# sshaoshuai/PointRCNN

Hardware: AMD Instinct MI355X
Metric: KITTI frames/sec, RPN inference end-to-end (16384 pts/frame, bs32 per GPU) (higher is better)
Workload: dtype f32 via split-bf16x6 MFMA (every fp32 operand cut exactly into 3 bf16 pieces, 6 bf16 MFMA products per fp32 product, fp32 accumulate: fp32-grade, measured error 2.9e-7 of sum|x||w| vs 3.0e-7 for the fp32-MFMA kernel; hoisted grouped layers on the split kernel too, unhoisted grouped first layers (xyz; 1 GPU; Full RPN PointNet++ backbone (4 SA-MSG + 4 FP) + cls/reg heads, tools/cfgs/default.yaml, 16384 pts/frame, batch 32 per GPU, random-init weights, eval-mode BN; frames_per_gpu=32, npoints=16384, parallelism=frames sharded, dp1, launch=hipGraph replay, streams=20, hw_queues=4, proposal_layer=normal, clouds=uniform, group_dedup=True, roi_dedup=True

## Files before the change

__graft_entry__.py:

```python
import os
import sys

ROOT = os.path.dirname(os.path.abspath(__file__))
if ROOT not in sys.path:
    sys.path.insert(0, ROOT)


def build():
    from pointrcnn_amd import build as hip_build
    hip_build.build(force=os.path.exists(hip_build.HIPCC), verbose=False)
    import pointrcnn_amd
    pointrcnn_amd.install()
    from pointrcnn_amd import _cabi
    lib = _cabi.lib()
    assert lib.prcnn_abi_version() >= 10
    import oracle
    oracle.build()
    from oracle import stage_reference
    if stage_reference.have_reference():
        stage_reference.stage()
    import pointnet2_lib.pointnet2.pointnet2_modules
    import iou3d_cuda, roipool3d_cuda, pointnet2_cuda


def smoke():
    import numpy as np
    import torch
    import pointrcnn_amd
    pointrcnn_amd.install()
    from pointrcnn_amd import _cabi, ops
    import oracle
    assert torch.cuda.is_available(), "smoke() needs a GPU"
    assert os.path.exists(_cabi.library_path()), "HIP extension missing"
    dev = torch.device("cuda:0")
    cpu = oracle.cpu()
    rng = np.random.default_rng(0)
    T = lambda a: torch.from_numpy(np.ascontiguousarray(a)).to(dev)

    xyz = rng.random((2, 2048, 3), dtype=np.float32)
    fidx = ops.furthest_point_sample(T(xyz), 256)
    assert np.array_equal(fidx.cpu().numpy(), cpu.fps(xyz, 256)), "fps mismatch"
    new_xyz = ops.gather_rows(T(xyz), fidx)
    ia, ib = ops.ball_query2(0.1, 16, 0.2, 32, T(xyz), new_xyz)
    nx = new_xyz.cpu().numpy()
    assert np.array_equal(ia.cpu().numpy(), cpu.ball_query(0.1, 16, xyz, nx)), "ball_query mismatch"
    assert np.array_equal(ib.cpu().numpy(), cpu.ball_query(0.2, 32, xyz, nx)), "ball_query2 mismatch"
    feat = rng.normal(size=(2, 2048, 8)).astype(np.float32)
    w = (rng.normal(size=(32, 11)) * 0.3).astype(np.float32)
# ... 69 lines not shown
```

include/prcnn_pointops.h:

```cpp
#ifndef PRCNN_POINTOPS_H
#define PRCNN_POINTOPS_H

#include <stddef.h>
#include <stdint.h>

#ifdef __cplusplus
extern "C" {
#endif

typedef void* prcnn_stream_t;

#define PRCNN_OK 0
#define PRCNN_EINVAL (-1)
#define PRCNN_EHIP (-2)
#define PRCNN_EUNSUPPORTED (-3)

int prcnn_abi_version(void);
const char* prcnn_last_error(void);
const char* prcnn_build_id(void);


int prcnn_fps(const float* xyz, int B, int N, int npoint, float* tmp, int32_t* idx, prcnn_stream_t stream);

int prcnn_fps_status(void);

#define PRCNN_FPS_ORDER_CANONICAL 0
#define PRCNN_FPS_ORDER_UPSTREAM 1
int prcnn_fps_order(const float* xyz, int B, int N, int npoint, int order, float* tmp, int32_t* idx, prcnn_stream_t stream);

#define PRCNN_ARITH_CANONICAL 0
#define PRCNN_ARITH_UPSTREAM 1
int prcnn_fps_mode(const float* xyz, int B, int N, int npoint, int order, int arith, float* tmp, int32_t* idx, prcnn_stream_t stream);
int prcnn_ball_query_arith(const float* xyz, const float* new_xyz, int B, int N, int M, float radius, int nsample, int arith,
                           int32_t* idx, prcnn_stream_t stream);
int prcnn_three_nn_arith(const float* unknown, const float* known, int B, int n, int m, int arith, float* dist2, int32_t* idx,
                         prcnn_stream_t stream);

int prcnn_gather(const float* feat, const int32_t* idx, int B, int C, int N, int M, float* out, prcnn_stream_t stream);
int prcnn_gather_grad(const float* grad_out, const int32_t* idx, int B, int C, int N, int M, float* grad_feat,
                      prcnn_stream_t stream);

int prcnn_gather_rows(const float* in_cl, int ld_in, const int32_t* idx, int B, int N, int M, int C, float* out,
                      prcnn_stream_t stream);

int prcnn_ball_query(const float* xyz, const float* new_xyz, int B, int N, int M, float radius, int nsample,
                     int32_t* idx, prcnn_stream_t stream);
int prcnn_ball_query2(const float* xyz, const float* new_xyz, int B, int N, int M, float radius_a, int nsample_a,
                      int32_t* idx_a, float radius_b, int nsample_b, int32_t* idx_b, prcnn_stream_t stream);

int prcnn_group(const float* feat, const int32_t* idx, int B, int C, int N, int M, int nsample, float* out,
                prcnn_stream_t stream);
int prcnn_group_grad(const float* grad_out, const int32_t* idx, int B, int C, int N, int M, int nsample,
                     float* grad_feat, prcnn_stream_t stream);

int prcnn_three_nn(const float* unknown, const float* known, int B, int n, int m, float* dist2, int32_t* idx,
// ... 211 lines not shown
```

pointrcnn_amd/_cabi.py:

```python
import ctypes
import os

from . import build as _build

_P = ctypes.c_void_p
_I = ctypes.c_int
_F = ctypes.c_float
_L = ctypes.c_int64
_Z = ctypes.c_size_t
_D = ctypes.c_double



class TrainSrc(ctypes.Structure):
    _fields_ = [("mode", _I), ("rows", _L), ("K", _I),
                ("in_", _P), ("ld_in", _I), ("pro_scale", _P), ("pro_shift", _P),
                ("xyz", _P), ("new_xyz", _P), ("idx", _P), ("feat", _P), ("ld_feat", _I),
                ("B", _I), ("N", _I), ("M", _I), ("ns", _I), ("C", _I),
                ("known", _P), ("idx3", _P), ("w3", _P), ("skip", _P), ("ld_known", _I), ("ld_skip", _I),
                ("n", _I), ("m", _I), ("C2", _I), ("C1", _I),
                ("mult", _P), ("rows_dev", _P), ("norm_rows", _L), ("seg_off", _P), ("seg_cnt", _P), ("row_grp", _P), ("groups", _I)]


class TrainLayer(ctypes.Structure):
    _fields_ = [("Nout", _I), ("W", _P), ("gamma", _P), ("beta", _P), ("eps", _F), ("momentum", _F),
                ("running_mean", _P), ("running_var", _P), ("y", _P), ("cst", _P), ("ld_c", _I), ("wpack", _P), ("wpack_t", _P),
                ("dW", _P), ("dgamma", _P), ("dbeta", _P)]


REQUIRED_ABI = 10

SIGNATURES = {
    "prcnn_abi_version": (_I, []),
    "prcnn_last_error": (ctypes.c_char_p, []),
    "prcnn_build_id": (ctypes.c_char_p, []),
    "prcnn_fps": (_I, [_P, _I, _I, _I, _P, _P, _P]),
    "prcnn_fps_status": (_I, []),
    "prcnn_fps_order": (_I, [_P, _I, _I, _I, _I, _P, _P, _P]),
    "prcnn_fps_mode": (_I, [_P, _I, _I, _I, _I, _I, _P, _P, _P]),
    "prcnn_ball_query_arith": (_I, [_P, _P, _I, _I, _I, _F, _I, _I, _P, _P]),
    "prcnn_three_nn_arith": (_I, [_P, _P, _I, _I, _I, _I, _P, _P, _P]),
    "prcnn_rpn_labels": (_I, [_P, _P, _P, _I, _I, _I, _F, _P, _P, _P]),
    "prcnn_gt_aug_edit": (_I, [_P, _P, _P, _P, _P, _F, _P, _P, _P, _I, _I, _I, _I, _P, _P, _P, _P, _P]),
    "prcnn_corner_iou3d": (_I, [_P, _I, _P, _I, _P, _P, _P]),
    "prcnn_gt_aug_sample": (_I, [_P, _P, _P, _I, _I, _P, _P, _P, _I, _P, _I, _P, _I, _P, _P, _I, _I, ctypes.c_uint32,
                                 _P, _P, _P, _P, _P, _P, _P, _P]),
    "prcnn_host_pts_in_boxes3d": (_I, [_P, _P, _L, _L, _P]),
    "prcnn_host_roipool3d": (_I, [_P, _P, _P, _L, _L, _L, _L, _P, _P, _P]),
    "prcnn_gather": (_I, [_P, _P, _I, _I, _I, _I, _P, _P]),
    "prcnn_gather_grad": (_I, [_P, _P, _I, _I, _I, _I, _P, _P]),
    "prcnn_gather_rows": (_I, [_P, _I, _P, _I, _I, _I, _I, _P, _P]),
    "prcnn_ball_query": (_I, [_P, _P, _I, _I, _I, _F, _I, _P, _P]),
    "prcnn_ball_query2": (_I, [_P, _P, _I, _I, _I, _F, _I, _P, _F, _I, _P, _P]),
    "prcnn_group": (_I, [_P, _P, _I, _I, _I, _I, _I, _P, _P]),
    "prcnn_group_grad": (_I, [_P, _P, _I, _I, _I, _I, _I, _P, _P]),
    "prcnn_three_nn": (_I, [_P, _P, _I, _I, _I, _P, _P, _P, _P]),
    "prcnn_three_interp": (_I, [_P, _P, _P, _I, _I, _I, _I, _P, _P]),
    "prcnn_three_interp_grad": (_I, [_P, _P, _P, _I, _I, _I, _I, _P, _P, _P]),
    "prcnn_wpack_floats": (_Z, [_I, _I]),
    "prcnn_pack_weight": (_I, [_P, _I, _I, _I, _P, _P]),
    "prcnn_mlp_rows": (_I, [_P, _I, _L, _I, _P, _P, _I, _I, _P, _I, _I, _I, _P, _I, _P, _I, _P]),
    "prcnn_mlp_group": (_I, [_P, _P, _P, _P, _I, _I, _I, _I, _I, _I, _P, _P, _P, _P, _I, _I, _P, _I, _I, _I, _P, _P]),
    "prcnn_mlp_group_split": (_I, [_P, _P, _P, _P, _I, _I, _I, _I, _I, _I, _P, _P, _P, _P, _I, _P, _I, _I, _P, _I, _I, _I, _P, _P]),
    "prcnn_mlp_interp": (_I, [_P, _I, _P, _P, _P, _I, _I, _I, _I, _I, _I, _P, _P, _P, _I, _I, _P, _I, _I, _P]),
    "prcnn_mlp_rows_addinterp": (_I, [_P, _I, _I, _P, _P, _I, _I, _P, _I, _P, _P, _I, _I, _I, _P, _I, _I, _P]),
    "prcnn_wsplit_bytes": (_Z, [_I, _I]),
    "prcnn_pack_weight_split": (_I, [_P, _I, _I, _I, _P, _P]),
    "prcnn_mlp_chain_interp_split": (_I, [_P, _I, _P, _P, _I, _I, _I, _I, _P, _P, _P, _P, _I, _I, _I, _P, _I, _I, _P]),
    "prcnn_mlp_chain_rows_split": (_I, [_P, _I, _L, _I, _P, _P, _P, _P, _P, _I, _P, _I, _I, _P]),
# ... 54 lines not shown
    pass


def library_path():
    return _build.LIB


def lib():
    global _lib
    if _lib is not None:
        return _lib
    import torch
    path = _build.LIB
    if not os.path.exists(path):
        try:
            _build.build(verbose=False)
        except Exception as e:
            raise PointOpsError(
                "libprcnn_pointops.so is missing and could not be built (%s). The HIP extension is "
                "mandatory: there is no CPU fallback. Run `python -m pointrcnn_amd.build`." % e)
    elif not os.environ.get("PRCNN_POINTOPS_LIB") and _build.have_sources() and _build.library_id(path) != _build.source_id():
        if not os.path.exists(_build.HIPCC):
            raise PointOpsError("%s is stale (built from %s, sources are %s) and hipcc is not available to rebuild it"
                                % (path, _build.library_id(path), _build.source_id()))
        try:
            _build.build(verbose=False)
        except Exception as e:
            raise PointOpsError("%s is stale and could not be rebuilt (%s)" % (path, e))
    try:
        handle = ctypes.CDLL(path)
    except OSError as e:
        raise PointOpsError("cannot load %s: %s" % (path, e))
    handle.prcnn_abi_version.restype = _I
    if handle.prcnn_abi_version() < REQUIRED_ABI:
        raise PointOpsError("%s implements ABI %d, this binding needs %d (include/prcnn_pointops.h)"
                            % (path, handle.prcnn_abi_version(), REQUIRED_ABI))
    for name, (res, args) in SIGNATURES.items():
        fn = getattr(handle, name)
        fn.restype = res
        fn.argtypes = args
    _lib = handle
    return handle


EUNSUPPORTED = -3


def check(rc, what=""):
    if rc != 0:
        msg = lib().prcnn_last_error()
        raise PointOpsError("%s failed (code %d): %s" % (what or "prcnn call", rc, msg.decode() if msg else "?"))
```

pointrcnn_amd/csrc/cabi_common.hip:

```cpp
#include "common.h"
#include <stdarg.h>

static thread_local char g_err[512] = "";

int prcnn_fail(int code, const char* fmt, ...) {
    va_list ap;
    va_start(ap, fmt);
    vsnprintf(g_err, sizeof(g_err), fmt, ap);
    va_end(ap);
    return code;
}

PRCNN_API const char* prcnn_last_error(void) { return g_err; }
PRCNN_API int prcnn_abi_version(void) { return 10; }

#ifndef PRCNN_BUILD_ID
#define PRCNN_BUILD_ID "PRCNN_BUILD_ID=unknown"
#endif
PRCNN_API const char* prcnn_build_id(void) { return &PRCNN_BUILD_ID[sizeof("PRCNN_BUILD_ID=") - 1]; }
```

pointrcnn_amd/csrc/fps.hip:

```cpp
#include "lds_sort.h"

typedef float f32x2 __attribute__((ext_vector_type(2)));
template <int PPT> struct fvec_t { typedef float type __attribute__((ext_vector_type(PPT))); };
template <> struct fvec_t<1> { typedef float type __attribute__((ext_vector_type(2))); };

#define FPS_DPP_MAX(v, ctrl) asm volatile("s_nop 1\n\tv_max_i32_dpp %0, %0, %0 " ctrl : "+v"(v))

__device__ __forceinline__ int wave_max_i32_fused(int v) {
    FPS_DPP_MAX(v, "row_shr:1 row_mask:0xf bank_mask:0xf");
    FPS_DPP_MAX(v, "row_shr:2 row_mask:0xf bank_mask:0xf");
    FPS_DPP_MAX(v, "row_shr:4 row_mask:0xf bank_mask:0xf");
    FPS_DPP_MAX(v, "row_shr:8 row_mask:0xf bank_mask:0xf");
    FPS_DPP_MAX(v, "row_bcast:15 row_mask:0xa bank_mask:0xf");
    FPS_DPP_MAX(v, "row_bcast:31 row_mask:0xc bank_mask:0xf");
    asm volatile("s_nop 1");
    return __builtin_amdgcn_readlane(v, 63);
}
__device__ __forceinline__ int row0_max_i32_fused(int v) {
    FPS_DPP_MAX(v, "row_shr:1 row_mask:0xf bank_mask:0xf");
    FPS_DPP_MAX(v, "row_shr:2 row_mask:0xf bank_mask:0xf");
    FPS_DPP_MAX(v, "row_shr:4 row_mask:0xf bank_mask:0xf");
    FPS_DPP_MAX(v, "row_shr:8 row_mask:0xf bank_mask:0xf");
    asm volatile("s_nop 1");
    return __builtin_amdgcn_readlane(v, 15);
// ... 73 lines not shown
                     "s_nop 1\n\t"
                     : [t] "=&v"(t), [acc] "=&v"(acc), [sa] "=&s"(sa), [sb] "=&s"(sb)
                     : [best] "v"(best), [p0] "v"(pt[0]), [p1] "v"(pt[1]), [p2] "v"(pt[2]), [p3] "v"(pt[3])
                     : "vcc");
        eqbits = acc;
        return t;
    }
};

#define FPS_EQ2(pa, pb) "v_cmp_eq_f32_e64 %[sa], " pa ", %[best]\n\tv_cmp_eq_f32_e64 %[sb], " pb ", %[best]\n\t"
#define FPS_AC2 "v_addc_co_u32_e64 %[a0], vcc, %[a0], %[a0], %[sa]\n\tv_addc_co_u32_e64 %[a1], vcc, %[a1], %[a1], %[sb]\n\t"
template <class V> __device__ __forceinline__ int wave_max_eq2_16(const V& pt, float best, unsigned& eqbits) {
    int t; unsigned a0, a1; unsigned long long sa, sb, sc, sd;
    asm volatile("v_mov_b32 %[t], %[best]\n\tv_mov_b32 %[a0], 0\n\tv_mov_b32 %[a1], 0\n\t"
                 FPS_EQ2("%[p15]", "%[p7]") FPS_D1 FPS_AC2
                 FPS_EQ2("%[p14]", "%[p6]") FPS_D2 FPS_AC2
                 FPS_EQ2("%[p13]", "%[p5]") FPS_D3 FPS_AC2
                 FPS_EQ2("%[p12]", "%[p4]") FPS_D4 FPS_AC2
                 FPS_EQ2("%[p11]", "%[p3]") FPS_D5 FPS_AC2
                 FPS_EQ2("%[p10]", "%[p2]") FPS_D6 FPS_AC2
                 FPS_EQ2("%[p9]", "%[p1]")
                 "v_cmp_eq_f32_e64 %[sc], %[p8], %[best]\n\tv_cmp_eq_f32_e64 %[sd], %[p0], %[best]\n\t"
                 FPS_AC2
                 "v_addc_co_u32_e64 %[a0], vcc, %[a0], %[a0], %[sc]\n\tv_addc_co_u32_e64 %[a1], vcc, %[a1], %[a1], %[sd]\n\t"
                 : [t] "=&v"(t), [a0] "=&v"(a0), [a1] "=&v"(a1), [sa] "=&s"(sa), [sb] "=&s"(sb), [sc] "=&s"(sc), [sd] "=&s"(sd)
                 : [best] "v"(best), [p0] "v"(pt[0]), [p1] "v"(pt[1]), [p2] "v"(pt[2]), [p3] "v"(pt[3]), [p4] "v"(pt[4]), [p5] "v"(pt[5]),
                   [p6] "v"(pt[6]), [p7] "v"(pt[7]), [p8] "v"(pt[8]), [p9] "v"(pt[9]), [p10] "v"(pt[10]), [p11] "v"(pt[11]),
                   [p12] "v"(pt[12]), [p13] "v"(pt[13]), [p14] "v"(pt[14]), [p15] "v"(pt[15])
                 : "vcc");
    eqbits = (a0 << 8) | a1;
    return t;
}

template <int BLOCK, int PPT>
__global__ __launch_bounds__(BLOCK) void fps_reg_kernel(const float* __restrict__ xyz, int N, int npoint,
                                                        int32_t* __restrict__ idx_out) {
    constexpr int NW = BLOCK / 64;
    typedef typename fvec_t<PPT>::type fvec;
    __shared__ float slot[2][NW][8];

    const int b = blockIdx.x;
    const int tid = threadIdx.x;
    const int lane = tid & 63;
    const int wave = tid >> 6;
    const float* __restrict__ p = xyz + (size_t)b * N * 3;
    int32_t* __restrict__ out = idx_out + (size_t)b * npoint;

    fvec px, py, pz, pt;
#pragma unroll
    for (int i = 0; i < PPT; i++) {
        int k = tid * PPT + i;
        bool ok = k < N;
        px[i] = ok ? p[k * 3 + 0] : 0.f;
        py[i] = ok ? p[k * 3 + 1] : 0.f;
        pz[i] = ok ? p[k * 3 + 2] : 0.f;
        pt[i] = ok ? 1e10f : -1.0f;
    }
    if (tid == 0 && npoint > 0) out[0] = 0;
    float x0 = p[0], y0 = p[1], z0 = p[2];

    for (int j = 1; j < npoint; j++) {
        float best = -2.0f;
        if (PPT >= 2) {
            const f32x2 qx = {x0, x0}, qy = {y0, y0}, qz = {z0, z0};
#pragma unroll
            for (int i = 0; i + 1 < PPT; i += 2) {
                f32x2 dx = (f32x2){px[i], px[i + 1]} - qx;
                f32x2 dy = (f32x2){py[i], py[i + 1]} - qy;
                f32x2 dz = (f32x2){pz[i], pz[i + 1]} - qz;
// ... 31 lines not shown
            }
            __syncthreads();
            const float* r = slot[j & 1][lane < NW ? lane : 0];
            int v = lane < NW ? __float_as_int(r[0]) : (int)0x80000000;
            int id = __float_as_int(r[1]);
            float rx = r[2], ry = r[3], rz = r[4];
            const int gmax = row0_max_i32_fused(v);
            const int wwin = __builtin_ctzll(__ballot(v == gmax));
            gidx = __builtin_amdgcn_readlane(id, wwin);
            x0 = __int_as_float(__builtin_amdgcn_readlane(__float_as_int(rx), wwin));
            y0 = __int_as_float(__builtin_amdgcn_readlane(__float_as_int(ry), wwin));
            z0 = __int_as_float(__builtin_amdgcn_readlane(__float_as_int(rz), wwin));
        }
        if (tid == 0) out[j] = gidx;
    }
}

#define FPS_BIG 1.0e18f
#ifndef FPS_V
#define FPS_V 6
#endif
#ifndef FPS_PAIR_ASM
#define FPS_PAIR_ASM 1
#endif

__device__ __forceinline__ unsigned morton_spread6(unsigned v) {
    v &= 0x3fu;
    v = (v | (v << 8)) & 0x0000300fu;
    v = (v | (v << 4)) & 0x000030c3u;
    v = (v | (v << 2)) & 0x00009249u;
    return v;
}

__global__ __launch_bounds__(1024) void fps_sort_kernel(const float* __restrict__ xyz, int N, int NP, int32_t* __restrict__ perm) {
    extern __shared__ unsigned keys[];
    __shared__ float red[6][16];
    const int b = blockIdx.x, tid = threadIdx.x, lane = tid & 63, wave = tid >> 6, nw = blockDim.x >> 6;
    const float* __restrict__ p = xyz + (size_t)b * N * 3;
    float lo[3] = {FPS_BIG, FPS_BIG, FPS_BIG}, hi[3] = {-FPS_BIG, -FPS_BIG, -FPS_BIG};
    for (int k = tid; k < N; k += blockDim.x)
#pragma unroll
        for (int a = 0; a < 3; a++) { float v = p[k * 3 + a]; lo[a] = fminf(lo[a], v); hi[a] = fmaxf(hi[a], v); }
#pragma unroll
    for (int a = 0; a < 3; a++) {
        for (int o = 32; o > 0; o >>= 1) { lo[a] = fminf(lo[a], __shfl_xor(lo[a], o)); hi[a] = fmaxf(hi[a], __shfl_xor(hi[a], o)); }
        if (lane == 0) { red[a][wave] = lo[a]; red[3 + a][wave] = hi[a]; }
    }
    __syncthreads();
    float scale[3];
#pragma unroll
    for (int a = 0; a < 3; a++) {
        float l = red[a][0], h = red[3 + a][0];
        for (int w = 1; w < nw; w++) { l = fminf(l, red[a][w]); h = fmaxf(h, red[3 + a][w]); }
        lo[a] = l;
        scale[a] = (h > l) ? 63.0f / (h - l) : 0.f;
    }
    unsigned v[16];
    if (tid * 16 < NP) {
#pragma unroll
        for (int e = 0; e < 16; e++) {
            const int k = tid * 16 + e;
            unsigned key = ~0u;
            if (k < N) {
                unsigned qx = (unsigned)((p[k * 3 + 0] - lo[0]) * scale[0]);
                unsigned qy = (unsigned)((p[k * 3 + 1] - lo[1]) * scale[1]);
                unsigned qz = (unsigned)((p[k * 3 + 2] - lo[2]) * scale[2]);
                unsigned m = (morton_spread6(qx) << 2) | (morton_spread6(qz) << 1) | morton_spread6(qy);
// ... 50 lines not shown
}
__device__ __forceinline__ void fps_xt_publish(unsigned (*xt)[64], int cb, int wave, const fps_cand_t& c) {
    unsigned* t = xt[cb];
    t[wave] = __float_as_uint(c.x); t[16 + wave] = __float_as_uint(c.y); t[32 + wave] = __float_as_uint(c.z);
    asm volatile("ds_max_u64 %0, %1 offset:192" : : "v"((unsigned)(size_t)&t[0]), "v"(c.key) : "memory");
    if (wave == 0) *(unsigned long long*)&xt[cb == 2 ? 0 : cb + 1][48] = 0ULL;
}
__device__ __forceinline__ int fps_xt_collect(unsigned (*xt)[64], int cb, int lane, float& x0, float& y0, float& z0, int& wl) {
    const int tv = (int)xt[cb][lane];
    const unsigned klo = (unsigned)__builtin_amdgcn_readlane(tv, 48);
    wl = (int)(klo & 15u);
    x0 = __int_as_float(__builtin_amdgcn_readlane(tv, wl));
    y0 = __int_as_float(__builtin_amdgcn_readlane(tv, wl | 16));
    z0 = __int_as_float(__builtin_amdgcn_readlane(tv, wl | 32));
    return (int)(0xFFFFFFFu - (klo >> 4));
}

#ifdef PRCNN_FPS_TIMING
__device__ unsigned long long prcnn_fps_dbg[16 * 8 + 16 + 16 * 16];
PRCNN_API int prcnn_fps_timing_read(unsigned long long* host_out) {
    return hipMemcpyFromSymbol(host_out, HIP_SYMBOL(prcnn_fps_dbg), sizeof(prcnn_fps_dbg)) == hipSuccess ? 0 : -1;
}
#define FPS_T(...) __VA_ARGS__
#ifndef PRCNN_FPS_TIMING_WAVE
#define PRCNN_FPS_TIMING_WAVE -1
#endif
#define FPS_NOW(w) ((PRCNN_FPS_TIMING_WAVE < 0 || (w) == PRCNN_FPS_TIMING_WAVE) ? __builtin_readcyclecounter() : 0ULL)
#else
#define FPS_T(...)
#endif

template <int PPT>
__global__ __launch_bounds__(1024) void fps_pruned_kernel(const float* __restrict__ xyz, const int32_t* __restrict__ perm,
                                                          int N, int npoint, int32_t* __restrict__ idx_out) {
    constexpr int BLOCK = 1024, NW = 16;
    typedef typename fvec_t<PPT>::type fvec;
    FPS_XT_DECL;
    extern __shared__ int s_po[];
    __builtin_amdgcn_s_setprio(2);

    const int b = blockIdx.x, tid = threadIdx.x, lane = tid & 63, wave = tid >> 6;
    const int wave_u = __builtin_amdgcn_readfirstlane(wave);
    const float* __restrict__ p = xyz + (size_t)b * N * 3;
    const int32_t* __restrict__ pm = perm + (size_t)b * N;
    int32_t* __restrict__ out = idx_out + (size_t)b * npoint;

    fvec px, py, pz, pt;
    float lox = FPS_BIG, loy = FPS_BIG, loz = FPS_BIG, hix = -FPS_BIG, hiy = -FPS_BIG, hiz = -FPS_BIG;
#pragma unroll
    for (int i = 0; i < PPT; i++) {
        int s = tid * PPT + i;
        bool ok = s < N;
        int o = ok ? pm[s] : 0x7fffffff;
        s_po[i * BLOCK + tid] = o;
        px[i] = ok ? p[o * 3 + 0] : 0.f;
        py[i] = ok ? p[o * 3 + 1] : 0.f;
        pz[i] = ok ? p[o * 3 + 2] : 0.f;
        pt[i] = ok ? 1e10f : -1.0f;
        if (ok) {
            lox = fminf(lox, px[i]); hix = fmaxf(hix, px[i]);
            loy = fminf(loy, py[i]); hiy = fmaxf(hiy, py[i]);
            loz = fminf(loz, pz[i]); hiz = fmaxf(hiz, pz[i]);
        }
    }
    lox = wave_min_f32_fused(lox); loy = wave_min_f32_fused(loy); loz = wave_min_f32_fused(loz);
    hix = wave_max_f32_fused(hix); hiy = wave_max_f32_fused(hiy); hiz = wave_max_f32_fused(hiz);

// ... 78 lines not shown
                cy = __int_as_float(__builtin_amdgcn_readlane(__float_as_int(by), owner));
                cz = __int_as_float(__builtin_amdgcn_readlane(__float_as_int(bz), owner));
            }
            cval = wmaxf;
            first = false;
            fps_cand_set(cand, wave, cx, cy, cz, cval, corig);
            FPS_T(t_u4 += __builtin_readcyclecounter() - u3;)
            }
            __builtin_amdgcn_s_setprio(2);
        }
#if FPS_V & 2
        else __builtin_amdgcn_s_setprio(2);
#endif
        FPS_T(unsigned long long t1 = __builtin_readcyclecounter(); t_upd += t1 - t0; n_upd += update ? 1 : 0;)
        if (lane == 0) fps_xt_publish(xt, cb, wave, cand);
        __syncthreads();
        FPS_T(unsigned long long t2 = __builtin_readcyclecounter(); t_wait += t2 - t1;)
        int wwin;
        const int gorig = fps_xt_collect(xt, cb, lane, x0, y0, z0, wwin);
#if FPS_V & 2
        if ((unsigned)(wave_u - wwin + 1) <= 2u) __builtin_amdgcn_s_setprio(3);
#endif
        wprev = wwin;
        cb = cb == 2 ? 0 : cb + 1;
        if (tid == 0) out[j] = gorig;
        FPS_T(t0 = __builtin_readcyclecounter(); t_red += t0 - t2;)
    }
    FPS_T(if (b == 0 && lane == 0) { unsigned long long* d = prcnn_fps_dbg + wave * 8; d[0] = t_upd; d[1] = t_wait; d[2] = t_red; d[3] = n_upd;
                                     d[4] = __builtin_readcyclecounter() - t_begin; d[5] = t_u1; d[6] = t_u2; d[7] = t_u3; prcnn_fps_dbg[128 + wave] = t_u4; })
}

template <int PPT, int NW>
__global__ __launch_bounds__(NW * 64) void fps_slot_kernel(const float* __restrict__ xyz, const int32_t* __restrict__ perm,
                                                          int N, int npoint, int32_t* __restrict__ idx_out) {
    constexpr int BLOCK = NW * 64;
    typedef typename fvec_t<PPT>::type fvec;
    FPS_XT_DECL;
    extern __shared__ int s_po[];
    __builtin_amdgcn_s_setprio(2);

    const int b = blockIdx.x, tid = threadIdx.x, lane = tid & 63, wave = tid >> 6;
    const int wave_u = __builtin_amdgcn_readfirstlane(wave);
    const float* __restrict__ p = xyz + (size_t)b * N * 3;
    const int32_t* __restrict__ pm = perm + (size_t)b * N;
    int32_t* __restrict__ out = idx_out + (size_t)b * npoint;

    fvec px, py, pz, pt;
    float lox = FPS_BIG, loy = FPS_BIG, loz = FPS_BIG, hix = -FPS_BIG, hiy = -FPS_BIG, hiz = -FPS_BIG;
#pragma unroll
    for (int i = 0; i < PPT; i++) {
        int s = (wave * PPT + i) * 64 + lane;
        bool ok = s < N;
        int o = ok ? pm[s] : 0x7fffffff;
        s_po[i * BLOCK + tid] = o;
        px[i] = ok ? p[o * 3 + 0] : 0.f;
        py[i] = ok ? p[o * 3 + 1] : 0.f;
        pz[i] = ok ? p[o * 3 + 2] : 0.f;
        pt[i] = ok ? 1e10f : -1.0f;
        if (ok) {
            lox = fminf(lox, px[i]); hix = fmaxf(hix, px[i]);
            loy = fminf(loy, py[i]); hiy = fmaxf(hiy, py[i]);
            loz = fminf(loz, pz[i]); hiz = fmaxf(hiz, pz[i]);
        }
    }
    lox = wave_min_f32_fused(lox); loy = wave_min_f32_fused(loy); loz = wave_min_f32_fused(loz);
    hix = wave_max_f32_fused(hix); hiy = wave_max_f32_fused(hiy); hiz = wave_max_f32_fused(hiz);

// ... 136 lines not shown
        }
#if FPS_V & 2
        else __builtin_amdgcn_s_setprio(2);
#endif
        FPS_T(unsigned long long q4 = FPS_NOW(wave);)
        if (lane == 0) fps_xt_publish(xt, cb, wave, cand);
        __syncthreads();
        FPS_T(unsigned long long q5 = FPS_NOW(wave); q_pub += q5 - q4;)
        int wwin;
        const int gorig = fps_xt_collect(xt, cb, lane, x0, y0, z0, wwin);
#if FPS_V & 2
        if ((unsigned)(wave_u - wwin + 1) <= 2u) __builtin_amdgcn_s_setprio(3);
#endif
        wprev = wwin;
        cb = cb == 2 ? 0 : cb + 1;
        if (tid == 0) out[j] = gorig;
        FPS_T(q0 = FPS_NOW(wave); q_coll += q0 - q5;)
    }
    FPS_T(if (b == 0 && lane == 0) { unsigned long long* d = prcnn_fps_dbg + 144 + wave * 16; d[0] = q_test; d[1] = q_dist; d[2] = q_max; d[3] = q_search; d[4] = q_pub;
                                     d[5] = q_coll; d[6] = q_nupd; d[7] = q_npair; d[8] = FPS_NOW(wave) - q_begin; })
}

struct fps_bcand_t { float x, y, z, v, s; unsigned orig, mask; unsigned long long key; };
__device__ __forceinline__ void fps_bcand_set(fps_bcand_t& c, int wave, float cx, float cy, float cz, float cval, float csec, int corig, unsigned cmask) {
    const unsigned hi = (unsigned)__float_as_int(cval) ^ 0x80000000u;
    const unsigned o = (unsigned)min(corig, 0xFFFFFFF);
    c.x = cx; c.y = cy; c.z = cz; c.v = cval; c.s = csec; c.orig = o; c.mask = cmask; c.key = ((unsigned long long)hi << 32) | ((0xFFFFFFFu - o) << 4) | (unsigned)wave;
    asm volatile("" : "+v"(c.x), "+v"(c.y), "+v"(c.z), "+v"(c.v), "+v"(c.s), "+v"(c.orig), "+v"(c.mask), "+v"(c.key));
}
#define FPS_BT_WORDS 160

template <int PPT, int NW>
__global__ __launch_bounds__(NW * 64) void fps_batch_kernel(const float* __restrict__ xyz, const int32_t* __restrict__ perm,
                                                           int N, int npoint, int32_t* __restrict__ idx_out) {
    static_assert(NW == 16 && PPT == 16, "rows of 16 lanes = the 16 waves; 8 pair boxes");
    constexpr int BLOCK = NW * 64;
    typedef typename fvec_t<PPT>::type fvec;
    typedef float f32x4 __attribute__((ext_vector_type(4)));
    typedef unsigned u32x4 __attribute__((ext_vector_type(4)));
    __shared__ __attribute__((aligned(256))) unsigned xt[3][FPS_BT_WORDS];
    __shared__ __attribute__((aligned(32))) float wbox[16][8];
    extern __shared__ int s_po[];
    __builtin_amdgcn_s_setprio(2);

    const int b = blockIdx.x, tid = threadIdx.x, lane = tid & 63, wave = tid >> 6, l15 = lane & 15;
    const int wave_u = __builtin_amdgcn_readfirstlane(wave);
    const float* __restrict__ p = xyz + (size_t)b * N * 3;
    const int32_t* __restrict__ pm = perm + (size_t)b * N;
    int32_t* __restrict__ out = idx_out + (size_t)b * npoint;

    fvec px, py, pz, pt;
    float lox = FPS_BIG, loy = FPS_BIG, loz = FPS_BIG, hix = -FPS_BIG, hiy = -FPS_BIG, hiz = -FPS_BIG;
#pragma unroll
    for (int i = 0; i < PPT; i++) {
        int s = (wave * PPT + i) * 64 + lane;
        bool ok = s < N;
        int o = ok ? pm[s] : 0x7fffffff;
        s_po[i * BLOCK + tid] = o;
        px[i] = ok ? p[o * 3 + 0] : 0.f;
        py[i] = ok ? p[o * 3 + 1] : 0.f;
        pz[i] = ok ? p[o * 3 + 2] : 0.f;
        pt[i] = ok ? 1e10f : -1.0f;
        if (ok) {
            lox = fminf(lox, px[i]); hix = fmaxf(hix, px[i]);
            loy = fminf(loy, py[i]); hiy = fmaxf(hiy, py[i]);
            loz = fminf(loz, pz[i]); hiz = fmaxf(hiz, pz[i]);
        }
// ... 294 lines not shown
    __shared__ int sval[2][NW], sidx[2][NW];
    const int b = blockIdx.x, tid = threadIdx.x, lane = tid & 63, wave = tid >> 6;
    const float* __restrict__ p = xyz + (size_t)b * N * 3;
    float* __restrict__ t = tmp + (size_t)b * N;
    int32_t* __restrict__ out = idx_out + (size_t)b * npoint;
    for (int k = tid; k < N; k += 1024) t[k] = 1e10f;
    if (tid == 0 && npoint > 0) out[0] = 0;
    int old = 0;
    for (int j = 1; j < npoint; j++) {
        float x0 = p[old * 3], y0 = p[old * 3 + 1], z0 = p[old * 3 + 2];
        float best = -2.0f;
        int bk = 0x7fffffff;
        for (int k = tid; k < N; k += 1024) {
            float d = sqdist3(p[k * 3], p[k * 3 + 1], p[k * 3 + 2], x0, y0, z0);
            float v = t[k];
            v = d < v ? d : v;
            t[k] = v;
            if (v > best) { best = v; bk = k; }
        }
        int vb = __float_as_int(best);
        int wmax = wave_max_i32(vb);
        int widx = wave_min_i32(vb == wmax ? bk : 0x7fffffff);
        if (lane == 0) { sval[j & 1][wave] = wmax; sidx[j & 1][wave] = widx; }
        __syncthreads();
        int v = lane < NW ? sval[j & 1][lane] : (int)0x80000000;
        int id = lane < NW ? sidx[j & 1][lane] : 0x7fffffff;
        int gmax = row0_max_i32(v);
        old = row0_min_i32(v == gmax ? id : 0x7fffffff);
        if (tid == 0) out[j] = old;
    }
}

template <int BLOCK, int PPT>
static void launch_fps(const float* xyz, int B, int N, int npoint, int32_t* idx, hipStream_t s) {
    hipLaunchKernelGGL((fps_reg_kernel<BLOCK, PPT>), dim3(B), dim3(BLOCK), 0, s, xyz, N, npoint, idx);
}

static int* fps_timeout_word() {
    static int* word = [] {
        int* w = nullptr;
        if (hipHostMalloc((void**)&w, sizeof(int), hipHostMallocMapped) != hipSuccess) { (void)hipGetLastError(); return (int*)nullptr; }
        *w = 0;
        return w;
    }();
    return word;
}

PRCNN_API int prcnn_fps_status(void) {
    int* w = fps_timeout_word();
    if (w && __atomic_exchange_n(w, 0, __ATOMIC_RELAXED) != 0)
        return prcnn_fail(PRCNN_EHIP, "prcnn_fps: a multi-workgroup launch (N > 16384) gave up waiting for a partner slice; "
                                      "its output holds -1 indices (were all ceil(N/16384) workgroups of a frame able to become resident?)");
    return PRCNN_OK;
}

PRCNN_API int prcnn_fps(const float* xyz, int B, int N, int npoint, float* tmp, int32_t* idx, prcnn_stream_t stream) {
    PRCNN_REQUIRE(B >= 0 && N > 0 && npoint >= 0, "prcnn_fps: bad shape B=%d N=%d npoint=%d", B, N, npoint);
    PRCNN_REQUIRE(npoint <= N, "prcnn_fps: npoint %d > N %d", npoint, N);
    if (B == 0 || npoint == 0) return PRCNN_OK;
    PRCNN_REQUIRE(xyz && idx, "prcnn_fps: null pointer");
    hipStream_t s = (hipStream_t)stream;
    if (tmp && N > 2048 && N <= 16384) {
        int NP = 1;
        while (NP < N) NP <<= 1;
        int32_t* perm = reinterpret_cast<int32_t*>(tmp);
        static PrcnnLdsLimit sort_attr;
        if (!sort_attr.raise((const void*)fps_sort_kernel, 80 * 1024))
            return prcnn_fail(PRCNN_EHIP, "prcnn_fps: cannot raise the dynamic LDS limit of the sort kernel");
        const int sort_threads = NP / 16 < 64 ? 64 : NP / 16;
        hipLaunchKernelGGL(fps_sort_kernel, dim3(B), dim3(sort_threads), lds_sort_bytes(NP, sizeof(unsigned)), s, xyz, N, NP, perm);
        PRCNN_LAUNCH_CHECK("prcnn_fps(sort)");
        static PrcnnLdsLimit pruned_attr;
        if (!pruned_attr.raise((const void*)fps_pruned_kernel<16>, 16 * 4096))
            return prcnn_fail(PRCNN_EHIP, "prcnn_fps: cannot raise the dynamic LDS limit of the pruned kernel");
        const char* slots_env = getenv("PRCNN_FPS_SLOTS");
        const bool slots = slots_env == nullptr || atoi(slots_env) != 0;
        static PrcnnLdsLimit slot_attr;
        if (slots && N > 8192 && !slot_attr.raise((const void*)fps_slot_kernel<16, 16>, 16 * 4096))
            return prcnn_fail(PRCNN_EHIP, "prcnn_fps: cannot raise the dynamic LDS limit of the slot kernel");
        const char* batch_env = getenv("PRCNN_FPS_BATCH");
        const bool batch = batch_env != nullptr && atoi(batch_env) != 0;
        static PrcnnLdsLimit batch_attr;
        if (slots && batch && N > 8192 && !batch_attr.raise((const void*)fps_batch_kernel<16, 16>, 16 * 4096))
            return prcnn_fail(PRCNN_EHIP, "prcnn_fps: cannot raise the dynamic LDS limit of the batch kernel");
        if (slots && batch && N > 8192) hipLaunchKernelGGL((fps_batch_kernel<16, 16>), dim3(B), dim3(1024), 16 * 4096, s, xyz, perm, N, npoint, idx);
        else if (slots && N > 8192) hipLaunchKernelGGL((fps_slot_kernel<16, 16>), dim3(B), dim3(1024), 16 * 4096, s, xyz, perm, N, npoint, idx);
        else if (N <= 4096) hipLaunchKernelGGL((fps_pruned_kernel<4>), dim3(B), dim3(1024), 4 * 4096, s, xyz, perm, N, npoint, idx);
        else if (N <= 8192) hipLaunchKernelGGL((fps_pruned_kernel<8>), dim3(B), dim3(1024), 8 * 4096, s, xyz, perm, N, npoint, idx);
        else hipLaunchKernelGGL((fps_pruned_kernel<16>), dim3(B), dim3(1024), 16 * 4096, s, xyz, perm, N, npoint, idx);
    }
    else if (N <= 64) launch_fps<64, 1>(xyz, B, N, npoint, idx, s);
    else if (N <= 128) launch_fps<64, 2>(xyz, B, N, npoint, idx, s);
    else if (N <= 256) launch_fps<64, 4>(xyz, B, N, npoint, idx, s);
    else if (N <= 512) launch_fps<64, 8>(xyz, B, N, npoint, idx, s);
    else if (N <= 1024) launch_fps<64, 16>(xyz, B, N, npoint, idx, s);
    else if (N <= 2048) launch_fps<256, 8>(xyz, B, N, npoint, idx, s);
    else if (N <= 4096) launch_fps<256, 16>(xyz, B, N, npoint, idx, s);
    else if (N <= 8192) launch_fps<1024, 8>(xyz, B, N, npoint, idx, s);
    else if (N <= 16384) launch_fps<1024, 16>(xyz, B, N, npoint, idx, s);
    else {
        PRCNN_REQUIRE(tmp, "prcnn_fps: N=%d > 16384 needs the (B,N) tmp buffer", N);
        const int S = prcnn_divup(N, FPS_MULTI_SLICE);
        static const bool use_mem = getenv("PRCNN_FPS_MEM") != nullptr;
        if (!use_mem && S <= FPS_MULTI_MAX_SPLIT && ((uintptr_t)tmp & 7) == 0) {
            const size_t slot_bytes = (size_t)B * 2 * S * 5 * sizeof(unsigned long long);
            if (prcnn_fill_words(tmp, 0xFFFFFFFFu, slot_bytes / 4, s) != hipSuccess) return prcnn_fail(PRCNN_EHIP, "prcnn_fps: cannot clear the exchange slots");
            if (int st = prcnn_fps_status()) return st;
            hipLaunchKernelGGL(fps_multi_kernel, dim3(B * S), dim3(1024), 0, s, xyz, N, npoint, S, reinterpret_cast<unsigned long long*>(tmp), idx,
                               fps_timeout_word());
        } else {
            hipLaunchKernelGGL(fps_mem_kernel, dim3(B), dim3(1024), 0, s, xyz, N, npoint, tmp, idx);
        }
    }
    PRCNN_LAUNCH_CHECK("prcnn_fps");
    return PRCNN_OK;
}

__global__ __launch_bounds__(1024) void fps_upstream_order_kernel(const float* __restrict__ xyz, int N, int npoint, int T,
                                                                  float* __restrict__ tmp, int32_t* __restrict__ idx_out) {
    constexpr int NWMAX = 16;
    __shared__ int sval[2][NWMAX], stid[2][NWMAX], sidx[2][NWMAX];
    const int b = blockIdx.x, tid = threadIdx.x, lane = tid & 63, wave = tid >> 6;
    const int nw = (blockDim.x + 63) >> 6;
    const float* __restrict__ p = xyz + (size_t)b * N * 3;
    float* __restrict__ t = tmp + (size_t)b * N;
    int32_t* __restrict__ out = idx_out + (size_t)b * npoint;
    for (int k = tid; k < N; k += blockDim.x) t[k] = 1e10f;
    if (tid == 0 && npoint > 0) out[0] = 0;
    __syncthreads();
    int old = 0;
    for (int j = 1; j < npoint; j++) {
        const float x0 = p[old * 3], y0 = p[old * 3 + 1], z0 = p[old * 3 + 2];
        float best = -2.0f;
        int bk = 0x7fffffff;
        if (tid < T) {
            for (int k = tid; k < N; k += T) {
                const float d = sqdist3(p[k * 3], p[k * 3 + 1], p[k * 3 + 2], x0, y0, z0);
                float v = t[k];
                v = d < v ? d : v;
                t[k] = v;
                if (v > best) { best = v; bk = k; }
            }
        }
        const int vb = __float_as_int(best);
        const int wmax = wave_max_i32(vb);
        const int wtid = wave_min_i32(vb == wmax ? tid : 0x7fffffff);
        const int wk = __shfl(bk, wtid & 63);
        if (lane == 0) { sval[j & 1][wave] = wmax; stid[j & 1][wave] = wtid; sidx[j & 1][wave] = wk; }
// ... 26 lines not shown
```

pointrcnn_amd/ops.py:

```python
import ctypes
import os
import threading

import torch

from . import _cabi

_INT = torch.int32
_F32 = torch.float32
FPS_PRUNED = os.environ.get("PRCNN_FPS_PRUNED", "1") == "1"


def _stream():
    return torch.cuda.current_stream().cuda_stream


def _chk(t, name, dtype=_F32, ndim=None):
    if not isinstance(t, torch.Tensor):
        raise TypeError("%s must be a torch.Tensor" % name)
    if not t.is_cuda:
        raise RuntimeError("%s must be a CUDA(HIP) tensor: the HIP kernels are the only implementation" % name)
    if t.dtype != dtype:
        raise RuntimeError("%s must have dtype %s, got %s" % (name, dtype, t.dtype))
    if not t.is_contiguous():
        raise RuntimeError("%s must be contiguous" % name)
    if ndim is not None and t.dim() != ndim:
        raise RuntimeError("%s must have %d dims, got shape %s" % (name, ndim, tuple(t.shape)))
    return t


def _p(t):
    return None if t is None else t.data_ptr()


def furthest_point_sample(xyz, npoint, order="canonical"):
    _chk(xyz, "xyz", ndim=3)
    B, N, _ = xyz.shape
    idx = torch.empty((B, npoint), dtype=_INT, device=xyz.device)
    if order != "canonical":
        if order != "upstream":
            raise ValueError("furthest_point_sample: order must be 'canonical' or 'upstream'")
        tmp = torch.empty((B, N), dtype=_F32, device=xyz.device)
        _cabi.check(_cabi.lib().prcnn_fps_order(_p(xyz), B, N, npoint, 1, _p(tmp), _p(idx), _stream()), "prcnn_fps_order")
        return idx
    tmp = torch.empty((B, N), dtype=_F32, device=xyz.device) if (N > 16384 or (N > 2048 and FPS_PRUNED)) else None
    L = _cabi.lib()
    _cabi.check(L.prcnn_fps(_p(xyz), B, N, npoint, _p(tmp), _p(idx), _stream()), "prcnn_fps")
    return idx


_ARITH = {"canonical": 0, "upstream": 1}
_ORDER = {"canonical": 0, "upstream": 1}


def furthest_point_sample_mode(xyz, npoint, order="canonical", arith="canonical"):
    _chk(xyz, "xyz", ndim=3)
    B, N, _ = xyz.shape
    idx = torch.empty((B, npoint), dtype=_INT, device=xyz.device)
    tmp = torch.empty((B, N), dtype=_F32, device=xyz.device)
    _cabi.check(_cabi.lib().prcnn_fps_mode(_p(xyz), B, N, npoint, _ORDER[order], _ARITH[arith], _p(tmp), _p(idx), _stream()), "prcnn_fps_mode")
    return idx


def ball_query_arith(radius, nsample, xyz, new_xyz, arith="upstream"):
    _chk(xyz, "xyz", ndim=3); _chk(new_xyz, "new_xyz", ndim=3)
    B, N, _ = xyz.shape
    M = new_xyz.shape[1]
    idx = torch.empty((B, M, nsample), dtype=_INT, device=xyz.device)
    _cabi.check(_cabi.lib().prcnn_ball_query_arith(_p(xyz), _p(new_xyz), B, N, M, float(radius), nsample, _ARITH[arith], _p(idx), _stream()),
                "prcnn_ball_query_arith")
    return idx


def three_nn_arith(unknown, known, arith="upstream"):
    _chk(unknown, "unknown", ndim=3); _chk(known, "known", ndim=3)
    B, n, _ = unknown.shape
    m = known.shape[1]
    d2 = torch.empty((B, n, 3), dtype=_F32, device=unknown.device)
    idx = torch.empty((B, n, 3), dtype=_INT, device=unknown.device)
    _cabi.check(_cabi.lib().prcnn_three_nn_arith(_p(unknown), _p(known), B, n, m, _ARITH[arith], _p(d2), _p(idx), _stream()),
                "prcnn_three_nn_arith")
    return d2, idx


def fps_status():
    _cabi.check(_cabi.lib().prcnn_fps_status(), "prcnn_fps_status")


def gather(features, idx):
    _chk(features, "features", ndim=3); _chk(idx, "idx", _INT, 2)
    B, C, N = features.shape
    M = idx.shape[1]
    out = torch.empty((B, C, M), dtype=_F32, device=features.device)
    _cabi.check(_cabi.lib().prcnn_gather(_p(features), _p(idx), B, C, N, M, _p(out), _stream()), "prcnn_gather")
    return out


def gather_grad(grad_out, idx, N):
    _chk(grad_out, "grad_out", ndim=3); _chk(idx, "idx", _INT, 2)
    B, C, M = grad_out.shape
    g = torch.zeros((B, C, N), dtype=_F32, device=grad_out.device)
    _cabi.check(_cabi.lib().prcnn_gather_grad(_p(grad_out), _p(idx), B, C, N, M, _p(g), _stream()), "prcnn_gather_grad")
    return g


def gather_rows(in_cl, idx):
    _chk(idx, "idx", _INT, 2)
    B, N, C = in_cl.shape
    M = idx.shape[1]
    out = torch.empty((B, M, C), dtype=_F32, device=in_cl.device)
    _cabi.check(_cabi.lib().prcnn_gather_rows(_p(in_cl), _row_stride(in_cl), _p(idx), B, N, M, C, _p(out), _stream()),
                "prcnn_gather_rows")
    return out


GRID_MIN_POINTS = 2048 if os.environ.get("PRCNN_GRID_SEARCH", "1") != "0" else 1 << 62
THREE_NN_GRID_MIN = int(os.environ.get("PRCNN_THREE_NN_GRID_MIN", "1024")) if GRID_MIN_POINTS < (1 << 62) else 1 << 62
DENSE_SCAN = os.environ.get("PRCNN_DENSE_SCAN", "1") != "0"
BQ_GRID_CELLS = int(os.environ.get("PRCNN_BQ_GRID_CELLS", "128"))


class Grid:

    def __init__(self, xyz, min_cell=0.0, cells_per_axis=64):
        _chk(xyz, "xyz", ndim=3)
        self.B, self.N = xyz.shape[0], xyz.shape[1]
        L = _cabi.lib()
        nbytes = L.prcnn_grid_bytes(self.B, self.N)
        self.buf = torch.empty((max(nbytes, 16),), dtype=torch.uint8, device=xyz.device)
        _cabi.check(L.prcnn_grid_build(_p(xyz), self.B, self.N, float(min_cell), int(cells_per_axis), _p(self.buf), nbytes, _stream()),
                    "prcnn_grid_build")


def ball_query_grid(grid, new_xyz, radius_a, nsample_a, radius_b=0.0, nsample_b=0, xyz=None):
    _chk(new_xyz, "new_xyz", ndim=3)
    B, M = new_xyz.shape[0], new_xyz.shape[1]
    if B != grid.B:
        raise ValueError("ball_query_grid: %d frames of centroids vs %d frames in the grid" % (B, grid.B))
    ia = torch.empty((B, M, nsample_a), dtype=_INT, device=new_xyz.device)
    ib = torch.empty((B, M, nsample_b), dtype=_INT, device=new_xyz.device) if nsample_b else None
    _cabi.check(_cabi.lib().prcnn_ball_query2_grid(_p(grid.buf), _p(xyz), _p(new_xyz), B, grid.N, M, float(radius_a), nsample_a, _p(ia),
                                                   float(radius_b), nsample_b, _p(ib), _stream()), "prcnn_ball_query2_grid")
    return (ia, ib) if nsample_b else ia


# ... 723 lines not shown
```

Before: 13870 frames/s.

## Skip nested FPS on already FPS-ordered inputs via a prefix validity check

Sampled xyz produced by gather_rows from an FPS index is tagged as FPS-ordered. A later furthest-point sample on such a set takes a nested path. A parallel prefix kernel writes the identity order, checks each point's minimum distance to earlier points for zeros or out-of-range values, and sets a per-frame flag. The existing FPS kernels read the flag and return early for frames whose prefix passed, which avoids the sequential FPS loop on the deeper SA levels. The cost is an extra kernel, a flag fill, and reliance on tagging that is tied to tensor versions.

```diff
diff --git a/__graft_entry__.py b/__graft_entry__.py
--- a/__graft_entry__.py
+++ b/__graft_entry__.py
@@ -13,7 +13,7 @@
     pointrcnn_amd.install()
     from pointrcnn_amd import _cabi
     lib = _cabi.lib()
-    assert lib.prcnn_abi_version() >= 10
+    assert lib.prcnn_abi_version() >= 11
     import oracle
     oracle.build()
     from oracle import stage_reference
diff --git a/include/prcnn_pointops.h b/include/prcnn_pointops.h
--- a/include/prcnn_pointops.h
+++ b/include/prcnn_pointops.h
@@ -21,6 +21,8 @@
 
 
 int prcnn_fps(const float* xyz, int B, int N, int npoint, float* tmp, int32_t* idx, prcnn_stream_t stream);
+
+int prcnn_fps_nested(const float* xyz, int B, int N, int npoint, float* tmp, int32_t* flags, int32_t* idx, prcnn_stream_t stream);
 
 int prcnn_fps_status(void);
 
diff --git a/pointrcnn_amd/_cabi.py b/pointrcnn_amd/_cabi.py
--- a/pointrcnn_amd/_cabi.py
+++ b/pointrcnn_amd/_cabi.py
@@ -29,12 +29,14 @@
 
 
 REQUIRED_ABI = 10
+ABI_SINCE = {"prcnn_fps_nested": 11}
 
 SIGNATURES = {
     "prcnn_abi_version": (_I, []),
     "prcnn_last_error": (ctypes.c_char_p, []),
     "prcnn_build_id": (ctypes.c_char_p, []),
     "prcnn_fps": (_I, [_P, _I, _I, _I, _P, _P, _P]),
+    "prcnn_fps_nested": (_I, [_P, _I, _I, _I, _P, _P, _P, _P]),
     "prcnn_fps_status": (_I, []),
     "prcnn_fps_order": (_I, [_P, _I, _I, _I, _I, _P, _P, _P]),
     "prcnn_fps_mode": (_I, [_P, _I, _I, _I, _I, _I, _P, _P, _P]),
@@ -155,9 +157,10 @@
     except OSError as e:
         raise PointOpsError("cannot load %s: %s" % (path, e))
     handle.prcnn_abi_version.restype = _I
-    if handle.prcnn_abi_version() < REQUIRED_ABI:
+    need = max([REQUIRED_ABI] + list(ABI_SINCE.values()))
+    if handle.prcnn_abi_version() < need:
         raise PointOpsError("%s implements ABI %d, this binding needs %d (include/prcnn_pointops.h)"
-                            % (path, handle.prcnn_abi_version(), REQUIRED_ABI))
+                            % (path, handle.prcnn_abi_version(), need))
     for name, (res, args) in SIGNATURES.items():
         fn = getattr(handle, name)
         fn.restype = res
diff --git a/pointrcnn_amd/csrc/cabi_common.hip b/pointrcnn_amd/csrc/cabi_common.hip
--- a/pointrcnn_amd/csrc/cabi_common.hip
+++ b/pointrcnn_amd/csrc/cabi_common.hip
@@ -12,7 +12,7 @@
 }
 
 PRCNN_API const char* prcnn_last_error(void) { return g_err; }
-PRCNN_API int prcnn_abi_version(void) { return 10; }
+PRCNN_API int prcnn_abi_version(void) { return 11; }
 
 #ifndef PRCNN_BUILD_ID
 #define PRCNN_BUILD_ID "PRCNN_BUILD_ID=unknown"
diff --git a/pointrcnn_amd/csrc/fps.hip b/pointrcnn_amd/csrc/fps.hip
--- a/pointrcnn_amd/csrc/fps.hip
+++ b/pointrcnn_amd/csrc/fps.hip
@@ -129,9 +129,12 @@
     return t;
 }
 
+#define FPS_SKIP_FRAME(skip) do { if ((skip) != nullptr && (skip)[blockIdx.x] != 0) return; } while (0)
+
 template <int BLOCK, int PPT>
 __global__ __launch_bounds__(BLOCK) void fps_reg_kernel(const float* __restrict__ xyz, int N, int npoint,
-                                                        int32_t* __restrict__ idx_out) {
+                                                        int32_t* __restrict__ idx_out, const int32_t* __restrict__ skip) {
+    FPS_SKIP_FRAME(skip);
     constexpr int NW = BLOCK / 64;
     typedef typename fvec_t<PPT>::type fvec;
     __shared__ float slot[2][NW][8];
@@ -229,7 +232,9 @@
     return v;
 }
 
-__global__ __launch_bounds__(1024) void fps_sort_kernel(const float* __restrict__ xyz, int N, int NP, int32_t* __restrict__ perm) {
+__global__ __launch_bounds__(1024) void fps_sort_kernel(const float* __restrict__ xyz, int N, int NP, int32_t* __restrict__ perm,
+                                                        const int32_t* __restrict__ skip) {
+    FPS_SKIP_FRAME(skip);
     extern __shared__ unsigned keys[];
     __shared__ float red[6][16];
     const int b = blockIdx.x, tid = threadIdx.x, lane = tid & 63, wave = tid >> 6, nw = blockDim.x >> 6;
@@ -346,7 +351,9 @@
 
 template <int PPT>
 __global__ __launch_bounds__(1024) void fps_pruned_kernel(const float* __restrict__ xyz, const int32_t* __restrict__ perm,
-                                                          int N, int npoint, int32_t* __restrict__ idx_out) {
+                                                          int N, int npoint, int32_t* __restrict__ idx_out,
+                                                          const int32_t* __restrict__ skip) {
+    FPS_SKIP_FRAME(skip);
     constexpr int BLOCK = 1024, NW = 16;
     typedef typename fvec_t<PPT>::type fvec;
     FPS_XT_DECL;
@@ -491,7 +498,9 @@
 
 template <int PPT, int NW>
 __global__ __launch_bounds__(NW * 64) void fps_slot_kernel(const float* __restrict__ xyz, const int32_t* __restrict__ perm,
-                                                          int N, int npoint, int32_t* __restrict__ idx_out) {
+                                                          int N, int npoint, int32_t* __restrict__ idx_out,
+                                                          const int32_t* __restrict__ skip) {
+    FPS_SKIP_FRAME(skip);
     constexpr int BLOCK = NW * 64;
     typedef typename fvec_t<PPT>::type fvec;
     FPS_XT_DECL;
@@ -694,7 +703,9 @@
 
 template <int PPT, int NW>
 __global__ __launch_bounds__(NW * 64) void fps_batch_kernel(const float* __restrict__ xyz, const int32_t* __restrict__ perm,
-                                                           int N, int npoint, int32_t* __restrict__ idx_out) {
+                                                           int N, int npoint, int32_t* __restrict__ idx_out,
+                                                           const int32_t* __restrict__ skip) {
+    FPS_SKIP_FRAME(skip);
     static_assert(NW == 16 && PPT == 16, "rows of 16 lanes = the 16 waves; 8 pair boxes");
     constexpr int BLOCK = NW * 64;
     typedef typename fvec_t<PPT>::type fvec;
@@ -1055,8 +1066,8 @@
 }
 
 template <int BLOCK, int PPT>
-static void launch_fps(const float* xyz, int B, int N, int npoint, int32_t* idx, hipStream_t s) {
-    hipLaunchKernelGGL((fps_reg_kernel<BLOCK, PPT>), dim3(B), dim3(BLOCK), 0, s, xyz, N, npoint, idx);
+static void launch_fps(const float* xyz, int B, int N, int npoint, int32_t* idx, const int32_t* skip, hipStream_t s) {
+    hipLaunchKernelGGL((fps_reg_kernel<BLOCK, PPT>), dim3(B), dim3(BLOCK), 0, s, xyz, N, npoint, idx, skip);
 }
 
 static int* fps_timeout_word() {
@@ -1077,7 +1088,7 @@
     return PRCNN_OK;
 }
 
-PRCNN_API int prcnn_fps(const float* xyz, int B, int N, int npoint, float* tmp, int32_t* idx, prcnn_stream_t stream) {
+static int fps_launch(const float* xyz, int B, int N, int npoint, float* tmp, int32_t* idx, const int32_t* skip, prcnn_stream_t stream) {
     PRCNN_REQUIRE(B >= 0 && N > 0 && npoint >= 0, "prcnn_fps: bad shape B=%d N=%d npoint=%d", B, N, npoint);
     PRCNN_REQUIRE(npoint <= N, "prcnn_fps: npoint %d > N %d", npoint, N);
     if (B == 0 || npoint == 0) return PRCNN_OK;
@@ -1091,7 +1102,7 @@
         if (!sort_attr.raise((const void*)fps_sort_kernel, 80 * 1024))
             return prcnn_fail(PRCNN_EHIP, "prcnn_fps: cannot raise the dynamic LDS limit of the sort kernel");
         const int sort_threads = NP / 16 < 64 ? 64 : NP / 16;
-        hipLaunchKernelGGL(fps_sort_kernel, dim3(B), dim3(sort_threads), lds_sort_bytes(NP, sizeof(unsigned)), s, xyz, N, NP, perm);
+        hipLaunchKernelGGL(fps_sort_kernel, dim3(B), dim3(sort_threads), lds_sort_bytes(NP, sizeof(unsigned)), s, xyz, N, NP, perm, skip);
         PRCNN_LAUNCH_CHECK("prcnn_fps(sort)");
         static PrcnnLdsLimit pruned_attr;
         if (!pruned_attr.raise((const void*)fps_pruned_kernel<16>, 16 * 4096))
@@ -1106,21 +1117,21 @@
         static PrcnnLdsLimit batch_attr;
         if (slots && batch && N > 8192 && !batch_attr.raise((const void*)fps_batch_kernel<16, 16>, 16 * 4096))
             return prcnn_fail(PRCNN_EHIP, "prcnn_fps: cannot raise the dynamic LDS limit of the batch kernel");
-        if (slots && batch && N > 8192) hipLaunchKernelGGL((fps_batch_kernel<16, 16>), dim3(B), dim3(1024), 16 * 4096, s, xyz, perm, N, npoint, idx);
-        else if (slots && N > 8192) hipLaunchKernelGGL((fps_slot_kernel<16, 16>), dim3(B), dim3(1024), 16 * 4096, s, xyz, perm, N, npoint, idx);
-        else if (N <= 4096) hipLaunchKernelGGL((fps_pruned_kernel<4>), dim3(B), dim3(1024), 4 * 4096, s, xyz, perm, N, npoint, idx);
-        else if (N <= 8192) hipLaunchKernelGGL((fps_pruned_kernel<8>), dim3(B), dim3(1024), 8 * 4096, s, xyz, perm, N, npoint, idx);
-        else hipLaunchKernelGGL((fps_pruned_kernel<16>), dim3(B), dim3(1024), 16 * 4096, s, xyz, perm, N, npoint, idx);
-    }
-    else if (N <= 64) launch_fps<64, 1>(xyz, B, N, npoint, idx, s);
-    else if (N <= 128) launch_fps<64, 2>(xyz, B, N, npoint, idx, s);
-    else if (N <= 256) launch_fps<64, 4>(xyz, B, N, npoint, idx, s);
-    else if (N <= 512) launch_fps<64, 8>(xyz, B, N, npoint, idx, s);
-    else if (N <= 1024) launch_fps<64, 16>(xyz, B, N, npoint, idx, s);
-    else if (N <= 2048) launch_fps<256, 8>(xyz, B, N, npoint, idx, s);
-    else if (N <= 4096) launch_fps<256, 16>(xyz, B, N, npoint, idx, s);
-    else if (N <= 8192) launch_fps<1024, 8>(xyz, B, N, npoint, idx, s);
-    else if (N <= 16384) launch_fps<1024, 16>(xyz, B, N, npoint, idx, s);
+        if (slots && batch && N > 8192) hipLaunchKernelGGL((fps_batch_kernel<16, 16>), dim3(B), dim3(1024), 16 * 4096, s, xyz, perm, N, npoint, idx, skip);
+        else if (slots && N > 8192) hipLaunchKernelGGL((fps_slot_kernel<16, 16>), dim3(B), dim3(1024), 16 * 4096, s, xyz, perm, N, npoint, idx, skip);
+        else if (N <= 4096) hipLaunchKernelGGL((fps_pruned_kernel<4>), dim3(B), dim3(1024), 4 * 4096, s, xyz, perm, N, npoint, idx, skip);
+        else if (N <= 8192) hipLaunchKernelGGL((fps_pruned_kernel<8>), dim3(B), dim3(1024), 8 * 4096, s, xyz, perm, N, npoint, idx, skip);
+        else hipLaunchKernelGGL((fps_pruned_kernel<16>), dim3(B), dim3(1024), 16 * 4096, s, xyz, perm, N, npoint, idx, skip);
+    }
+    else if (N <= 64) launch_fps<64, 1>(xyz, B, N, npoint, idx, skip, s);
+    else if (N <= 128) launch_fps<64, 2>(xyz, B, N, npoint, idx, skip, s);
+    else if (N <= 256) launch_fps<64, 4>(xyz, B, N, npoint, idx, skip, s);
+    else if (N <= 512) launch_fps<64, 8>(xyz, B, N, npoint, idx, skip, s);
+    else if (N <= 1024) launch_fps<64, 16>(xyz, B, N, npoint, idx, skip, s);
+    else if (N <= 2048) launch_fps<256, 8>(xyz, B, N, npoint, idx, skip, s);
+    else if (N <= 4096) launch_fps<256, 16>(xyz, B, N, npoint, idx, skip, s);
+    else if (N <= 8192) launch_fps<1024, 8>(xyz, B, N, npoint, idx, skip, s);
+    else if (N <= 16384) launch_fps<1024, 16>(xyz, B, N, npoint, idx, skip, s);
     else {
         PRCNN_REQUIRE(tmp, "prcnn_fps: N=%d > 16384 needs the (B,N) tmp buffer", N);
         const int S = prcnn_divup(N, FPS_MULTI_SLICE);
@@ -1137,6 +1148,58 @@
     }
     PRCNN_LAUNCH_CHECK("prcnn_fps");
     return PRCNN_OK;
+}
+
+PRCNN_API int prcnn_fps(const float* xyz, int B, int N, int npoint, float* tmp, int32_t* idx, prcnn_stream_t stream) {
+    return fps_launch(xyz, B, N, npoint, tmp, idx, nullptr, stream);
+}
+
+#define FPS_PREFIX_CHUNK 256
+__global__ __launch_bounds__(256) void fps_prefix_kernel(const float* __restrict__ xyz, int N, int npoint, int32_t* __restrict__ idx_out,
+                                                         int32_t* __restrict__ flags) {
+    __shared__ float sq[FPS_PREFIX_CHUNK * 3];
+    __shared__ float red[4][64];
+    const int b = blockIdx.y, tid = threadIdx.x, lane = tid & 63, wave = __builtin_amdgcn_readfirstlane(tid >> 6);
+    const int j0 = blockIdx.x * 64, j = j0 + lane;
+    const float* __restrict__ p = xyz + (size_t)b * N * 3;
+    const bool live = j < npoint;
+    const int jc = live ? j : 0;
+    const float jx = p[jc * 3 + 0], jy = p[jc * 3 + 1], jz = p[jc * 3 + 2];
+    float t = 1e10f;
+    const int iend = min(j0 + 64, npoint) - 1;
+    for (int c0 = 0; c0 < iend; c0 += FPS_PREFIX_CHUNK) {
+        const int n = min(FPS_PREFIX_CHUNK, iend - c0);
+        __syncthreads();
+        for (int k = tid; k < n * 3; k += 256) sq[k] = p[(size_t)c0 * 3 + k];
+        __syncthreads();
+        const int ie = min(wave * 64 + 64, n);
+        for (int ii = wave * 64; ii < ie; ii++) {
+            const float d = sqdist3(jx, jy, jz, sq[ii * 3 + 0], sq[ii * 3 + 1], sq[ii * 3 + 2]);
+            t = (c0 + ii < j) ? __builtin_fminf(t, d) : t;
+        }
+    }
+    red[wave][lane] = t;
+    __syncthreads();
+    if (wave == 0) {
+        t = __builtin_fminf(__builtin_fminf(red[0][lane], red[1][lane]), __builtin_fminf(red[2][lane], red[3][lane]));
+        const unsigned bits = __float_as_uint(t);
+        const bool bad = live && j > 0 && (bits - 1u) >= (0x501502F9u - 1u);
+        if (live) idx_out[(size_t)b * npoint + j] = j;
+        if (__ballot(bad) != 0 && lane == 0) flags[b] = 0;
+    }
+}
+
+PRCNN_API int prcnn_fps_nested(const float* xyz, int B, int N, int npoint, float* tmp, int32_t* flags, int32_t* idx, prcnn_stream_t stream) {
+    PRCNN_REQUIRE(B >= 0 && N > 0 && npoint >= 0 && npoint <= N, "prcnn_fps_nested: bad shape B=%d N=%d npoint=%d", B, N, npoint);
+    if (B == 0 || npoint == 0) return PRCNN_OK;
+    PRCNN_REQUIRE(xyz && idx && flags, "prcnn_fps_nested: null pointer");
+    hipStream_t s = (hipStream_t)stream;
+    const bool shortcut = N <= 16384;
+    if (prcnn_fill_words(flags, shortcut ? 1u : 0u, (size_t)B, s) != hipSuccess) return prcnn_fail(PRCNN_EHIP, "prcnn_fps_nested: cannot set the flags");
+    if (!shortcut) return fps_launch(xyz, B, N, npoint, tmp, idx, nullptr, stream);
+    hipLaunchKernelGGL(fps_prefix_kernel, dim3(prcnn_divup(npoint, 64), B), dim3(256), 0, s, xyz, N, npoint, idx, flags);
+    PRCNN_LAUNCH_CHECK("prcnn_fps_nested(prefix)");
+    return fps_launch(xyz, B, N, npoint, tmp, idx, flags, stream);
 }
 
 __global__ __launch_bounds__(1024) void fps_upstream_order_kernel(const float* __restrict__ xyz, int N, int npoint, int T,
diff --git a/pointrcnn_amd/ops.py b/pointrcnn_amd/ops.py
--- a/pointrcnn_amd/ops.py
+++ b/pointrcnn_amd/ops.py
@@ -1,6 +1,7 @@
 import ctypes
 import os
 import threading
+import weakref
 
 import torch
 
@@ -9,6 +10,9 @@
 _INT = torch.int32
 _F32 = torch.float32
 FPS_PRUNED = os.environ.get("PRCNN_FPS_PRUNED", "1") == "1"
+FPS_NESTED = os.environ.get("PRCNN_FPS_NESTED", "1") == "1"
+_FPS_TAG = "_prcnn_fps_ordered"
+_FPS_SRC = "_prcnn_fps_src"
 
 
 def _stream():
@@ -45,8 +49,18 @@
         return idx
     tmp = torch.empty((B, N), dtype=_F32, device=xyz.device) if (N > 16384 or (N > 2048 and FPS_PRUNED)) else None
     L = _cabi.lib()
-    _cabi.check(L.prcnn_fps(_p(xyz), B, N, npoint, _p(tmp), _p(idx), _stream()), "prcnn_fps")
+    if FPS_NESTED and fps_ordered(xyz):
+        flags = torch.empty((B,), dtype=_INT, device=xyz.device)
+        _cabi.check(L.prcnn_fps_nested(_p(xyz), B, N, npoint, _p(tmp), _p(flags), _p(idx), _stream()), "prcnn_fps_nested")
+        idx._prcnn_fps_flags = flags
+    else:
+        _cabi.check(L.prcnn_fps(_p(xyz), B, N, npoint, _p(tmp), _p(idx), _stream()), "prcnn_fps")
+    setattr(idx, _FPS_SRC, (weakref.ref(xyz), xyz._version))
     return idx
+
+
+def fps_ordered(xyz):
+    return getattr(xyz, _FPS_TAG, None) == xyz._version and xyz.dim() == 3 and xyz.shape[2] == 3
 
 
 _ARITH = {"canonical": 0, "upstream": 1}
@@ -111,6 +125,9 @@
     out = torch.empty((B, M, C), dtype=_F32, device=in_cl.device)
     _cabi.check(_cabi.lib().prcnn_gather_rows(_p(in_cl), _row_stride(in_cl), _p(idx), B, N, M, C, _p(out), _stream()),
                 "prcnn_gather_rows")
+    src = getattr(idx, _FPS_SRC, None)
+    if src is not None and C == 3 and src[0]() is in_cl and src[1] == in_cl._version and idx._version == 0:
+        setattr(out, _FPS_TAG, out._version)
     return out
 
 
```

Measured after the change: 14180 frames/s, median of 6. 2.2% higher.
